# shivangchopra11/MedMoE

Hardware: AMD Instinct MI355X
Metric: image-text pairs/sec at global batch 1024 (higher is better)
Workload: dtype bf16; 1 GPU; cfg2: ViT-B/16 + 12-layer text tower (frozen), 8 experts top-2, 224x224x3 + 77 tokens, fwd+bwd+clip+Adam; global_batch=1024, per_gpu_batch=1024, parallelism=dp1

## Files before the change

### medmoe_amd/csrc/gemm.hip

```cpp
#include "common.h"
#include "det_plan.h"
#include <utility>

#define BM 128
#define BN 128
#define BK 64

__device__ __attribute__((aligned(256))) bf16_t g_zero_page[2048];

struct GemmNTArgs {
  const bf16_t* A; const bf16_t* B; void* C;
  const float* bias; const bf16_t* residual; bf16_t* aux;
  const int* a_rowmap; const int* c_rowmap; const int4* tiles; const int* tile_count;
  long long strideB; long long strideBias;
  int M, N, K, lda, ldb, ldc, ldr, ldaux;
  int n_tiles_n, max_tiles_m;
  float alpha; int epi; int out_f32; int col_perm;
  const int* m_dev;
};

static int g_use_nt256 = 1, g_use_nt512 = 1, g_use_tn512 = 1, g_tn_rows = 1024, g_nt_max_grid = 256, g_use_scores512 = 1, g_use_nt4w = 1, g_use_tn4w = 1, g_tn_min_rows = 2048, g_tn_rows4w = 0, g_scores_skip_epi = 0;
#ifdef NT_EXPERIMENT
__device__ int g_nt_dbg_skip = 0;
#define NT_X(...) __VA_ARGS__
#else
#define NT_X(...)
#endif
#ifdef NT_TIMING
__device__ unsigned long long g_nt_timing[8 * 8];
#define NT_T(...) __VA_ARGS__
__device__ __forceinline__ long long nt_clk() {
  __builtin_amdgcn_sched_barrier(0); const long long c = clock64(); __builtin_amdgcn_sched_barrier(0); return c;
}
#else
#define NT_T(...)
#endif
extern int g_attn_resident;
extern int g_sa_rows;
extern int g_attn_rt13;
static int g_last_nt_kernel = -1;
extern "C" int medmoe_last_gemm_nt_kernel() { return g_last_nt_kernel; }
extern int g_ln_one_row;
int g_use_nt_direct = 1;
extern "C" int medmoe_set_option(int key, int value) {
  if (key == 16) { g_ln_one_row = value; return MM_OK; }
  if (key == 17) { g_use_nt_direct = value; return MM_OK; }
  if (key == 1) { g_use_nt256 = value; return MM_OK; }
  if (key == 2) { g_use_nt512 = value; return MM_OK; }
  if (key == 3) { g_use_tn512 = value; return MM_OK; }
  if (key == 4 && value >= 256) { g_tn_rows = value; return MM_OK; }
  if (key == 5 && value >= 1 && value <= 256) { g_nt_max_grid = value; return MM_OK; }
  if (key == 6) { g_use_scores512 = value; return MM_OK; }
  if (key == 7) { g_use_nt4w = value; return MM_OK; }
  if (key == 8) { g_use_tn4w = value; return MM_OK; }
  if (key == 9 && value >= 64) { g_tn_min_rows = value; return MM_OK; }
  if (key == 12) { g_scores_skip_epi = value; return MM_OK; }
  if (key == 15 && (value == 0 || value == 448 || value == 512)) { g_attn_rt13 = value; return MM_OK; }
  if (key == 13 && value >= 0) { g_sa_rows = value; return MM_OK; }
  if (key == 11) { g_attn_resident = value; return MM_OK; }
  if (key == 10 && value >= 0) { g_tn_rows4w = value; return MM_OK; }
  return MM_ERR_ARG;
}

enum { EPI_NONE = 0, EPI_GELU = 1, EPI_RELU = 2, EPI_MUL_DGELU = 3, EPI_MUL_DRELU = 4, EPI_GELU_DAUX = 5, EPI_MUL_AUX = 6 };

struct ParkedTile {
  uint4 c[8];
  int m_base, n_base, n_items, next;
};

typedef unsigned u32x4e_t __attribute__((ext_vector_type(4)));
template <bool PARK, int TM0 = 0, int TMS = 4, int TN0 = 0, int TNS = 4, bool LDSX = false>
__device__ __forceinline__ int nt_epilogue(const GemmNTArgs& p, f32x4_t (&acc)[TMS][TNS], int m_base, int m_end,
                                           int n_base, int group, int frag_row, int frag_q, ParkedTile* park, unsigned lds_x = 0u) {
  int n_stores = 0;
  const int pg = ((frag_q & 1) << 1) | (frag_q >> 1);
  long long mc[4];
  bool mok[4];
#pragma unroll
  for (int tm = 0; tm < 4; ++tm) {
    const int m = m_base + tm * 16 + frag_row;
    mok[tm] = m < m_end;
    const int mr = min(m, m_end - 1);
    mc[tm] = p.c_rowmap ? (long long)p.c_rowmap[mr] : (long long)mr;
  }
  int nn[4];
  bool nok[4];
#pragma unroll
  for (int tn = 0; tn < 4; ++tn) {
    const int n = n_base + tn * 16 + pg * 4;
    nok[tn] = n < p.N;
    nn[tn] = min(n, p.N - 4);
// ... 1985 lines not shown
  for (int u = 0; u < U; ++u) {
    compute();
    if (grp == 0) { wait_third_newest(); seg_barrier(); }
    if (grp == 1) seg_barrier();
    load_seg();
  }
  if (grp == 0) seg_barrier();

  float* dW = p.dW + (MAPPED ? (long long)group * p.strideW : 0ll);
  const int kcol = lane & 31;
#pragma unroll
  for (int tn = 0; tn < 4; ++tn)
#pragma unroll
    for (int tk = 0; tk < 2; ++tk) {
      const int k = k0 + wn * 64 + tk * 32 + kcol;
#pragma unroll
      for (int r = 0; r < 16; ++r) {
        const int n = n0 + wm * 128 + tn * 32 + (r & 3) + 8 * (r >> 2) + 4 * h;
        if (!MAPPED || n < p.Nn) atomicAdd(dW + (long long)n * p.ldw + k, acc[tn][tk][r]);
      }
    }
  if (do_db) {
#pragma unroll
    for (int tn = 0; tn < 4; ++tn) {
      const float v = colsum[tn] + __shfl_xor(colsum[tn], 32, 64);
      const int n = n0 + wm * 128 + tn * 32 + kcol;
      if (h == 0 && (!MAPPED || n < p.Nn)) atomicAdd(p.db + (MAPPED ? (long long)group * p.strideDb : 0ll) + n, v);
    }
  }
}

typedef unsigned u32x4_t __attribute__((ext_vector_type(4)));
#define W_READ(dst, addr, imm) asm volatile("ds_read_b128 %0, %1 offset:%2" : "=v"(dst) : "v"(addr), "n"(imm))
template <bool MAPPED, bool COLG = false, bool SCALE = false>
__global__ __launch_bounds__(256) void gemm_tn4w_kernel(GemmTNArgs p) {
  static_assert(!(MAPPED && COLG), "column groups only in the plain build");
  static_assert(!SCALE || COLG, "row weights only in the column-group build");
  __shared__ __attribute__((aligned(128))) char smem[4 * SUB3 + (MAPPED ? 32768 : 0) + (SCALE ? 4096 : 0)];
  const int tid = threadIdx.x, lane = tid & 63, wid = __builtin_amdgcn_readfirstlane(tid >> 6);
  const int wm = wid & 1, wn = wid >> 1;
  int id = xcd_remap(blockIdx.x, gridDim.x);
  const int ntile = p.tiles_n * p.tiles_k;
  int group = 0, ms, me;
  if (MAPPED && p.row_off) {
    const int tile = id % ntile;
    if (!det_plan::tn_group_range(p.row_off, p.n_groups, p.nsplit, id / ntile, group, ms, me)) return;
    id = tile;
  } else {
    if (COLG) { group = id / (ntile * p.nsplit); id -= group * ntile * p.nsplit; }
    const int split = id / ntile; id -= split * ntile;
    det_plan::tn_split_range(p.M, p.nsplit, split, ms, me);
  }
  const int tile_n = id / p.tiles_k, tile_k = id - tile_n * p.tiles_k;
  if (ms >= me) return;
  const int U = (me - ms + 31) / 32;
  const int tail = (me - ms) - (U - 1) * 32;
  const int n0 = tile_n * 256, k0 = tile_k * 256;

  const int prow = (wid << 1) + (lane >> 5);
  const unsigned lds0 = (unsigned)(size_t)smem;
  unsigned col_g, col_x;
  {
    const int lc0 = (lane & 31) ^ ((prow & 3) << 2);
    const int gcol = n0 + lc0 * 8;
    col_g = (unsigned)(((MAPPED || COLG) && gcol >= p.Nn) ? n0 : gcol) * 2u;
    if (COLG && p.g_chunk_w > 0) {
      const int gc = (gcol >= p.Nn) ? n0 : gcol;
      const int c0 = n0 / p.g_chunk_w, cc = gc / p.g_chunk_w;
      col_g = (unsigned)((long long)(cc - c0) * p.g_chunk_stride + (gc - cc * p.g_chunk_w)) * 2u;
    }
    const int xcol = k0 + lc0 * 8;
    col_x = (unsigned)((COLG && xcol >= p.Kk) ? k0 : xcol) * 2u;
  }
  const int* rmap = MAPPED ? (p.g_rowmap ? p.g_rowmap : p.x_rowmap) : nullptr;
  int* lmap = (int*)(smem + 4 * SUB3);
  if (MAPPED && rmap) {
    for (int i = tid; i < min(me - ms, 8192); i += 256) lmap[i] = rmap[ms + i];
    __syncthreads();
  }
  const unsigned ldg2 = (unsigned)p.ldg * 2u, ldx2 = (unsigned)p.ldx * 2u;
  int lk = 0, wb = 0, rb = 0;
  unsigned sg[4], sx[4];
  const char* gbase = (const char*)p.G + (COLG ? (long long)group * p.gcol_stride * 2 : 0ll)
                      + ((COLG && p.g_chunk_w > 0) ? (long long)(n0 / p.g_chunk_w) * p.g_chunk_stride * 2 : 0ll);
  const char* xbase = (const char*)p.X + (COLG ? (long long)group * p.xcol_stride * 2 : 0ll);
  const char* gsub = gbase;
  const char* xsub = xbase;
  const char* wbase = SCALE ? (const char*)(p.gscale + (long long)group * p.gscale_gstride) : nullptr;
  const char* wsub = wbase;
  int wr0 = 0;
  const unsigned wl0 = lds0 + 4 * SUB3 + wid * 1024;
  auto setup_rows = [&]() __attribute__((always_inline)) {
    if constexpr (!MAPPED) {
      const long long r0 = ms + min(lk, (me - ms) / 32 - 1) * 32;
      auto uni = [](const char* q) -> const char* {
        const unsigned long long v = (unsigned long long)q;
// ... 75 lines not shown
  };
  auto read_one = [&](Frags& f, unsigned bo, auto gc) __attribute__((always_inline)) {
    constexpr int g = decltype(gc)::value, t = (g >> 2) & 3, ks = (g >> 1) & 1, hi = g & 1;
    constexpr int off = ks * 8192 + hi * 2048;
    const unsigned a = aa[(g < 16 ? 0 : 4) + t] + bo;
    if constexpr (g < 16) { if constexpr (hi) TR_READ(f.gh[ks][t], a, off); else TR_READ(f.gl[ks][t], a, off); }
    else { if constexpr (hi) TR_READ(f.xh[ks][t], a, off); else TR_READ(f.xl[ks][t], a, off); }
  };
  auto frag = [&](u32x2_t lo, u32x2_t hi) -> bf16x8_t {
    const uint4 v = make_uint4(lo[0], lo[1], hi[0], hi[1]);
    return __builtin_bit_cast(bf16x8_t, v);
  };
  auto add_colsum = [&](Frags& f) __attribute__((always_inline)) {
    const s16x2_t ones = {(short)0x3F80, (short)0x3F80};
#pragma unroll
    for (int ks = 0; ks < 2; ++ks)
#pragma unroll
      for (int tn = 0; tn < 4; ++tn) {
        const uint4 v = __builtin_bit_cast(uint4, frag(f.gl[ks][tn], f.gh[ks][tn]));
        float c = colsum[tn];
        c = __builtin_amdgcn_fdot2_f32_bf16(__builtin_bit_cast(s16x2_t, v.x), ones, c, false);
        c = __builtin_amdgcn_fdot2_f32_bf16(__builtin_bit_cast(s16x2_t, v.y), ones, c, false);
        c = __builtin_amdgcn_fdot2_f32_bf16(__builtin_bit_cast(s16x2_t, v.z), ones, c, false);
        c = __builtin_amdgcn_fdot2_f32_bf16(__builtin_bit_cast(s16x2_t, v.w), ones, c, false);
        colsum[tn] = c;
      }
  };
  int u_now = 0;
  auto zero_tail = [&](int buf) __attribute__((always_inline)) {
    char* zb = smem + buf * SUB3;
    for (int z = tail * 32 + lane; z < 32 * 32; z += 64) *(uint4*)(zb + z * 16) = make_uint4(0, 0, 0, 0);
    asm volatile("s_waitcnt lgkmcnt(0)" ::: "memory");
  };
  auto substep = [&](Frags& c, Frags& n) __attribute__((always_inline)) {
    const unsigned bo = rb * SUB3;
    if (MAPPED && rmap && u_now >= 128 && (u_now & 127) == 0) {
      for (int i = tid; i < 4096; i += 256) {
        const int r = (u_now + 128) * 32 + i;
        if (r < me - ms) lmap[r & 8191] = rmap[ms + r];
      }
    }
    if (MAPPED && u_now + 1 == U - 1 && tail < 32) zero_tail(rb);
    if (do_db && (u_now & 1) == wn) add_colsum(c);
    auto one = [&](auto qc) __attribute__((always_inline)) {
      constexpr int qq = decltype(qc)::value, ks = qq >> 4, tn = (qq >> 2) & 3, tk = qq & 3;
      acc[tn][tk] = __builtin_amdgcn_mfma_f32_32x32x16_bf16(frag(c.gl[ks][tn], c.gh[ks][tn]), frag(c.xl[ks][tk], c.xh[ks][tk]), acc[tn][tk], 0, 0, 0);
      if constexpr (qq < 24) {
        __builtin_amdgcn_sched_barrier(0);
        if constexpr (qq < 8) { read_one(n, bo, std::integral_constant<int, 2 * qq>{}); read_one(n, bo, std::integral_constant<int, 2 * qq + 1>{}); }
        else read_one(n, bo, std::integral_constant<int, qq + 8>{});
        if constexpr (qq % 3 == 2) piece(qq / 3);
        if constexpr (SCALE && qq == 0) wpiece();
        if constexpr (SCALE && qq % 4 == 0) scale_frag(c, std::integral_constant<int, qq / 4 + 1>{});
        __builtin_amdgcn_sched_barrier(0);
      }
      if constexpr (SCALE && qq == 24) {
        __builtin_amdgcn_sched_barrier(0);
        scale_frag(c, std::integral_constant<int, 7>{});
        read_w(rb);
        __builtin_amdgcn_sched_barrier(0);
      }
      if constexpr (SCALE && qq == 28) {
        __builtin_amdgcn_sched_barrier(0);
        scale_frag(n, std::integral_constant<int, 0>{});
        __builtin_amdgcn_sched_barrier(0);
      }
// ... 58 lines not shown
      for (int tk = 0; tk < 4; ++tk)
#pragma unroll
        for (int r = 0; r < 16; ++r) part[((tn * 4 + tk) * 16 + r) * 64] = acc[tn][tk][r];
  } else {
#pragma unroll
  for (int tn = 0; tn < 4; ++tn)
#pragma unroll
    for (int tk = 0; tk < 4; ++tk) {
      const int k = k0 + wn * 128 + tk * 32 + kcol;
#pragma unroll
      for (int r = 0; r < 16; ++r) {
        const int n = n0 + wm * 128 + tn * 32 + (r & 3) + 8 * (r >> 2) + 4 * h;
        if ((!(MAPPED || COLG) || n < p.Nn) && (!COLG || k < p.Kk)) atomicAdd(dW + (long long)n * p.ldw + k, acc[tn][tk][r]);
      }
    }
  }
  if (do_db) {
    const bool db_staged = staged && p.db_partial != nullptr;
#pragma unroll
    for (int tn = 0; tn < 4; ++tn) {
      const float v = colsum[tn] + __shfl_xor(colsum[tn], 32, 64);
      const int n = n0 + wm * 128 + tn * 32 + kcol;
      if (db_staged) {
        if (h == 0) p.db_partial[((long long)pid << 9) + (wid << 7) + tn * 32 + kcol] = v;
      } else if (h == 0 && (!(MAPPED || COLG) || n < p.Nn)) atomicAdd(p.db + ((MAPPED || COLG) ? (long long)group * p.strideDb : 0ll) + n, v);
    }
  }
}

extern "C" int medmoe_gemm_tn(const void* G, int ldg, const void* X, int ldx, float* dW, int ldw, float* db, int M, int Nn, int Kk,
                              const int* x_rowmap, const int* g_rowmap, const int* row_off, int n_groups, long long strideW,
                              long long strideDb, int nsplit, hipStream_t stream);

__global__ __launch_bounds__(256) void tn_reduce_kernel(const float* __restrict__ partial, float* __restrict__ dW, int ldw, int ntile,
                                                        int tiles_k, int nvalid) {
  const int tile = blockIdx.x >> 6;
  const int e4 = (((blockIdx.x & 63) << 8) + threadIdx.x) << 2;
  float4 s = {0.f, 0.f, 0.f, 0.f};
  for (int sp = 0; sp < nvalid; ++sp) {
    const float4 v = *(const float4*)(partial + ((long long)(sp * ntile + tile) << 16) + e4);
    s.x += v.x; s.y += v.y; s.z += v.z; s.w += v.w;
  }
  const int lane = e4 & 63, r = (e4 >> 6) & 15, tk = (e4 >> 10) & 3, tn = (e4 >> 12) & 3, wid = e4 >> 14;
  const int wm = wid & 1, wn = wid >> 1, h = lane >> 5, kcol = lane & 31;
  const int tile_n = tile / tiles_k, tile_k = tile - tile_n * tiles_k;
  const int n = tile_n * 256 + wm * 128 + tn * 32 + (r & 3) + 8 * (r >> 2) + 4 * h;
  const int k = tile_k * 256 + wn * 128 + tk * 32 + kcol;
  float4* d = (float4*)(dW + (long long)n * ldw + k);
  float4 o = *d;
  o.x += s.x; o.y += s.y; o.z += s.z; o.w += s.w;
  *d = o;
}

struct TnReduceArgs {
  const float* partial; const float* db_partial; float* dW; float* db; const int* row_off;
  long long strideW, strideDb;
  int ldw, Nn, Kk, tiles_n, tiles_k, mode, nsplit, nvalid, n_groups, R, vec;
};
__global__ __launch_bounds__(256) void tn_reduce_det_kernel(TnReduceArgs p) {
  const int ntile = p.tiles_n * p.tiles_k;
  const int gt = blockIdx.x >> 6;
  const int group = gt / ntile, tile = gt - group * ntile;
  int first, count;
  if (p.mode == 0) { first = group * p.nsplit; count = p.nvalid; }
  else det_plan::tn_group_ranges(p.row_off, group, p.R, first, count);
  const int e4 = (((blockIdx.x & 63) << 8) + threadIdx.x) << 2;
  float4 s = {0.f, 0.f, 0.f, 0.f};
  for (int sp = 0; sp < count; ++sp) {
    const float4 v = *(const float4*)(p.partial + ((long long)((first + sp) * ntile + tile) << 16) + e4);
    s.x += v.x; s.y += v.y; s.z += v.z; s.w += v.w;
  }
  const int lane = e4 & 63, r = (e4 >> 6) & 15, tk = (e4 >> 10) & 3, tn = (e4 >> 12) & 3, wid = e4 >> 14;
  const int wm = wid & 1, wn = wid >> 1, h = lane >> 5, kcol = lane & 31;
  const int tile_n = tile / p.tiles_k, tile_k = tile - tile_n * p.tiles_k;
  const int n = tile_n * 256 + wm * 128 + tn * 32 + (r & 3) + 8 * (r >> 2) + 4 * h;
  const int k = tile_k * 256 + wn * 128 + tk * 32 + kcol;
  if (count > 0 && n < p.Nn && k < p.Kk) {
    float* d = p.dW + (long long)group * p.strideW + (long long)n * p.ldw + k;
    if (p.vec) {
      float4 o = *(float4*)d;
      o.x += s.x; o.y += s.y; o.z += s.z; o.w += s.w;
      *(float4*)d = o;
    } else { d[0] += s.x; d[1] += s.y; d[2] += s.z; d[3] += s.w; }
  }
  if (p.db && tile_k == 0 && (blockIdx.x & 63) == 0 && count > 0) {
    const int c = threadIdx.x;
    const int nn = tile_n * 256 + c;
    float a = 0.f;
    for (int sp = 0; sp < count; ++sp) {
      const float* q = p.db_partial + ((long long)((first + sp) * ntile + tile) << 9) + ((c >> 7) << 7) + (c & 127);
      a += q[0];
      a += q[256];
    }
    if (nn < p.Nn) p.db[(long long)group * p.strideDb + nn] += a;
  }
}

static inline bool tn_vec_ok(const float* dW, int ldw, long long strideW) {
  return ((unsigned long long)dW & 15) == 0 && (ldw % 4) == 0 && (strideW % 4) == 0;
}

extern "C" int medmoe_gemm_tn_staged(const void* G, int ldg, const void* X, int ldx, float* dW, int ldw, float* db, int M, int Nn, int Kk,
                                     float* scratch, long long scratch_floats, hipStream_t stream) {
  if (!G || !X || !dW) return MM_ERR_ARG;
  if (M <= 0 || Nn <= 0 || Kk <= 0 || (Nn % 8) || (Kk % 8) || (ldg % 8) || (ldx % 8)) return MM_ERR_SHAPE;
  const bool fit32 = (long long)M * ldg * 2 < (1ll << 32) && (long long)M * ldx * 2 < (1ll << 32);
  if (scratch && g_use_tn512 && g_use_tn4w && (M % 32) == 0 && (Nn % 256) == 0 && (Kk % 256) == 0 && M >= 4096 && fit32 && (ldw % 4) == 0) {
    GemmTNArgs p;
    p.partial = nullptr;
    p.G = (const bf16_t*)G; p.X = (const bf16_t*)X; p.dW = dW; p.db = db;
    p.x_rowmap = nullptr; p.g_rowmap = nullptr; p.row_off = nullptr; p.strideW = 0; p.strideDb = 0;
    p.M = M; p.Nn = Nn; p.Kk = Kk; p.ldg = ldg; p.ldx = ldx; p.ldw = ldw; p.gcol_stride = 0; p.xcol_stride = 0; p.g_chunk_w = 0; p.g_chunk_stride = 0;
    p.gscale = nullptr; p.gscale_gstride = 0; p.gscale_ld = 0;
    p.tiles_n = Nn / 256; p.tiles_k = Kk / 256;
    const int ntile = p.tiles_n * p.tiles_k;
    p.nsplit = max(1, min(256 / ntile, M / g_tn_min_rows));
    p.n_groups = 1;
    if (p.nsplit >= 2 && (long long)ntile * p.nsplit * 65536 <= scratch_floats) {
      p.partial = scratch;
      const int chunk = det_plan::tn_chunk(M, p.nsplit);
      const int nvalid = (M + chunk - 1) / chunk;
      const long long slots = (long long)ntile * p.nsplit;
      if (db && slots * (65536 + 512) <= scratch_floats) p.db_partial = scratch + slots * 65536;
      if (db && !p.db_partial) ++g_mm_nondet;
      hipLaunchKernelGGL(gemm_tn4w_kernel<false>, dim3(ntile * p.nsplit), dim3(256), 0, stream, p);
      if (p.db_partial) {
        TnReduceArgs q{scratch, p.db_partial, dW, db, nullptr, 0, 0, ldw, Nn, Kk, p.tiles_n, p.tiles_k, 0, p.nsplit, nvalid, 1, 0, 1};
        q.vec = tn_vec_ok(dW, ldw, 0);
        hipLaunchKernelGGL(tn_reduce_det_kernel, dim3(ntile * 64), dim3(256), 0, stream, q);
      } else {
        hipLaunchKernelGGL(tn_reduce_kernel, dim3(ntile * 64), dim3(256), 0, stream, scratch, dW, ldw, ntile, p.tiles_k, nvalid);
      }
      return mm_check_launch();
    }
  }
  return medmoe_gemm_tn(G, ldg, X, ldx, dW, ldw, db, M, Nn, Kk, nullptr, nullptr, nullptr, 1, 0, 0, 16, stream);
}

static int tn_cols_impl(const void* G, int ldg, const void* X, int ldx, float* dW, int ldw, int M, int Nn, int Kk,
                        int n_groups, long long gcol_stride, long long xcol_stride, long long strideW, int g_chunk_w,
                        long long g_chunk_stride, bool det, float* scratch, long long scratch_floats, hipStream_t stream) {
  if (!G || !X || !dW) return MM_ERR_ARG;
  if (M < 32 || (M % 32) || Nn <= 0 || Kk <= 0 || (Nn % 8) || (Kk % 8) || (ldg % 8) || (ldx % 8) || n_groups < 1) return MM_ERR_SHAPE;
  if ((gcol_stride % 8) || (xcol_stride % 8) || gcol_stride < 0 || xcol_stride < 0) return MM_ERR_SHAPE;
  if (32ll * ldg * 2 + 1024 >= (1ll << 32) || 32ll * ldx * 2 + 1024 >= (1ll << 32)) return MM_ERR_SHAPE;
  if ((g_chunk_w <= 0 && Nn > ldg) || Kk > ldx) return MM_ERR_SHAPE;
  if (g_chunk_w > 0 && ((g_chunk_w % 8) || g_chunk_w > ldg || (g_chunk_stride % 8) || g_chunk_stride < 0 ||
                        (256 / g_chunk_w + 2) * g_chunk_stride * 2 + 32ll * ldg * 2 >= (1ll << 32))) return MM_ERR_SHAPE;
  GemmTNArgs p;
  p.partial = nullptr;
  p.G = (const bf16_t*)G; p.X = (const bf16_t*)X; p.dW = dW; p.db = nullptr;
  p.x_rowmap = nullptr; p.g_rowmap = nullptr; p.row_off = nullptr; p.strideW = strideW; p.strideDb = 0;
  p.M = M; p.Nn = Nn; p.Kk = Kk; p.ldg = ldg; p.ldx = ldx; p.ldw = ldw;
  p.tiles_n = (Nn + 255) / 256; p.tiles_k = (Kk + 255) / 256;
  p.n_groups = n_groups; p.gcol_stride = gcol_stride; p.xcol_stride = xcol_stride;
  p.g_chunk_w = g_chunk_w; p.g_chunk_stride = g_chunk_stride;
  p.gscale = nullptr; p.partial = nullptr; p.gscale_gstride = 0; p.gscale_ld = 0;
  const long long ntile = (long long)p.tiles_n * p.tiles_k * n_groups;
  p.nsplit = (int)max(1ll, min(256ll / ntile, (long long)M / g_tn_min_rows));
  if (det && p.nsplit > 1) {
    if (!scratch || ntile * p.nsplit * 65536 > scratch_floats) return MM_ERR_ARG;
    p.partial = scratch;
    const int chunk = det_plan::tn_chunk(M, p.nsplit);
    hipLaunchKernelGGL((gemm_tn4w_kernel<false, true>), dim3((unsigned)(ntile * p.nsplit)), dim3(256), 0, stream, p);
    TnReduceArgs q{scratch, nullptr, dW, nullptr, nullptr, strideW, 0, ldw, Nn, Kk, p.tiles_n, p.tiles_k, 0, p.nsplit, (M + chunk - 1) / chunk,
                   n_groups, 0, tn_vec_ok(dW, ldw, strideW) ? 1 : 0};
    hipLaunchKernelGGL(tn_reduce_det_kernel, dim3((unsigned)(ntile * 64)), dim3(256), 0, stream, q);
    return mm_check_launch();
  }
  if (p.nsplit > 1) ++g_mm_nondet;
  hipLaunchKernelGGL((gemm_tn4w_kernel<false, true>), dim3((unsigned)(ntile * p.nsplit)), dim3(256), 0, stream, p);
  return mm_check_launch();
}

extern "C" int medmoe_gemm_tn_cols(const void* G, int ldg, const void* X, int ldx, float* dW, int ldw, int M, int Nn, int Kk,
                                   int n_groups, long long gcol_stride, long long xcol_stride, long long strideW, int g_chunk_w,
                                   long long g_chunk_stride, hipStream_t stream) {
  return tn_cols_impl(G, ldg, X, ldx, dW, ldw, M, Nn, Kk, n_groups, gcol_stride, xcol_stride, strideW, g_chunk_w, g_chunk_stride, false,
                      nullptr, 0, stream);
}

extern "C" int medmoe_gemm_tn_cols_det(const void* G, int ldg, const void* X, int ldx, float* dW, int ldw, int M, int Nn, int Kk,
                                       int n_groups, long long gcol_stride, long long xcol_stride, long long strideW, int g_chunk_w,
                                       long long g_chunk_stride, float* scratch, long long scratch_floats, hipStream_t stream) {
  return tn_cols_impl(G, ldg, X, ldx, dW, ldw, M, Nn, Kk, n_groups, gcol_stride, xcol_stride, strideW, g_chunk_w, g_chunk_stride, true,
                      scratch, scratch_floats, stream);
}

extern "C" long long medmoe_gemm_tn_cols_det_scratch(int M, int Nn, int Kk, int n_groups) {
  return det_plan::cols_scratch_floats(M, Nn, Kk, n_groups, g_tn_min_rows);
}

static int tn_gram_impl(const void* A, int lda, const float* w, long long w_gstride, int w_ld, float* dW, int ldw, int M,
                        int Nn, int n_groups, long long col_stride, long long strideW, bool det, hipStream_t stream) {
  if (!A || !w || !dW) return MM_ERR_ARG;
  if (M < 32 || (M % 32) || Nn <= 0 || (Nn % 8) || (lda % 8) || n_groups < 1 || Nn > lda || w_ld < 1 || w_gstride < 0) return MM_ERR_SHAPE;
  if ((col_stride % 8) || col_stride < 0 || 32ll * lda * 2 + 1024 >= (1ll << 32) || 64ll * w_ld * 4 >= (1ll << 32)) return MM_ERR_SHAPE;
  GemmTNArgs p;
  p.partial = nullptr;
  p.G = (const bf16_t*)A; p.X = (const bf16_t*)A; p.dW = dW; p.db = nullptr;
  p.x_rowmap = nullptr; p.g_rowmap = nullptr; p.row_off = nullptr; p.strideW = strideW; p.strideDb = 0;
  p.M = M; p.Nn = Nn; p.Kk = Nn; p.ldg = lda; p.ldx = lda; p.ldw = ldw;
  p.tiles_n = (Nn + 255) / 256; p.tiles_k = p.tiles_n;
  p.n_groups = n_groups; p.gcol_stride = col_stride; p.xcol_stride = col_stride;
  p.g_chunk_w = 0; p.g_chunk_stride = 0;
  p.gscale = w; p.gscale_gstride = w_gstride; p.gscale_ld = w_ld;
  const long long ntile = (long long)p.tiles_n * p.tiles_k * n_groups;
  p.nsplit = det ? 1 : (int)max(1ll, min(256ll / ntile, (long long)M / g_tn_min_rows));
  if (p.nsplit > 1) ++g_mm_nondet;
  hipLaunchKernelGGL((gemm_tn4w_kernel<false, true, true>), dim3((unsigned)(ntile * p.nsplit)), dim3(256), 0, stream, p);
  return mm_check_launch();
}

extern "C" int medmoe_gemm_tn_gram(const void* A, int lda, const float* w, long long w_gstride, int w_ld, float* dW, int ldw, int M,
                                   int Nn, int n_groups, long long col_stride, long long strideW, hipStream_t stream) {
  return tn_gram_impl(A, lda, w, w_gstride, w_ld, dW, ldw, M, Nn, n_groups, col_stride, strideW, false, stream);
}

extern "C" int medmoe_gemm_tn_gram_det(const void* A, int lda, const float* w, long long w_gstride, int w_ld, float* dW, int ldw, int M,
                                       int Nn, int n_groups, long long col_stride, long long strideW, hipStream_t stream) {
  return tn_gram_impl(A, lda, w, w_gstride, w_ld, dW, ldw, M, Nn, n_groups, col_stride, strideW, true, stream);
}

extern "C" int medmoe_gemm_tn(const void* G, int ldg, const void* X, int ldx, float* dW, int ldw,
                              float* db, int M, int Nn, int Kk, const int* x_rowmap,
                              const int* g_rowmap, const int* row_off, int n_groups, long long strideW,
                              long long strideDb, int nsplit, hipStream_t stream) {
  if (!G || !X || !dW) return MM_ERR_ARG;
  if (M <= 0 || Nn <= 0 || Kk <= 0 || (Nn % 8) || (Kk % 8) || (ldg % 8) || (ldx % 8)) return MM_ERR_SHAPE;
  if (n_groups < 1 || nsplit < 1) return MM_ERR_ARG;
  GemmTNArgs p;
  p.partial = nullptr;
  p.G = (const bf16_t*)G; p.X = (const bf16_t*)X; p.dW = dW; p.db = db;
  p.x_rowmap = x_rowmap; p.g_rowmap = g_rowmap; p.row_off = row_off; p.strideW = strideW; p.strideDb = strideDb;
  p.M = M; p.Nn = Nn; p.Kk = Kk; p.ldg = ldg; p.ldx = ldx; p.ldw = ldw; p.gcol_stride = 0; p.xcol_stride = 0; p.g_chunk_w = 0; p.g_chunk_stride = 0; p.gscale = nullptr; p.partial = nullptr; p.gscale_gstride = 0; p.gscale_ld = 0;
  const bool fit32 = (long long)M * ldg * 2 < (1ll << 32) && (long long)M * ldx * 2 < (1ll << 32);
  if (g_use_tn512 && !x_rowmap && !g_rowmap && !row_off && n_groups == 1 && (M % 32) == 0 && (Nn % 256) == 0 && (Kk % 256) == 0 &&
      M >= 4096 && fit32) {
    p.tiles_n = Nn / 256; p.tiles_k = Kk / 256;
    const int ntile = p.tiles_n * p.tiles_k;
    p.nsplit = max(1, min(256 / ntile, M / g_tn_min_rows));
    p.n_groups = 1;
    if (p.nsplit > 1) ++g_mm_nondet;
    if (g_use_tn4w) hipLaunchKernelGGL(gemm_tn4w_kernel<false>, dim3(ntile * p.nsplit), dim3(256), 0, stream, p);
    else hipLaunchKernelGGL(gemm_tn512_kernel<false>, dim3(ntile * p.nsplit), dim3(512), 0, stream, p);
    return mm_check_launch();
  }
  if (g_use_tn512 && !(x_rowmap && g_rowmap) && (Nn % 128) == 0 && (Kk % 256) == 0 && M / n_groups >= 4096 && fit32) {
    p.tiles_n = (Nn + 255) / 256; p.tiles_k = Kk / 256;
    const int ntile = p.tiles_n * p.tiles_k;
    p.n_groups = n_groups;
    ++g_mm_nondet;
    if (g_use_tn4w && row_off) {
      long long R = g_tn_rows4w > 0 ? (g_tn_rows4w + 31) / 32 * 32 : 4096;
      p.nsplit = (int)R;
      const int max_ranges = (int)(M / R) + n_groups;
      hipLaunchKernelGGL(gemm_tn4w_kernel<true>, dim3(ntile * max_ranges), dim3(256), 0, stream, p);
      return mm_check_launch();
    }
    p.nsplit = max(1, M / n_groups / g_tn_rows);
    if (g_use_tn4w) hipLaunchKernelGGL(gemm_tn4w_kernel<true>, dim3(ntile * p.nsplit * n_groups), dim3(256), 0, stream, p);
    else hipLaunchKernelGGL(gemm_tn512_kernel<true>, dim3(ntile * p.nsplit * n_groups), dim3(512), 0, stream, p);
    return mm_check_launch();
  }
  p.tiles_n = (Nn + 127) / 128; p.tiles_k = (Kk + 127) / 128; p.nsplit = nsplit; p.n_groups = n_groups;
  if (nsplit > 1) ++g_mm_nondet;
  const int grid = p.tiles_n * p.tiles_k * nsplit * n_groups;
  if (x_rowmap || g_rowmap) hipLaunchKernelGGL(gemm_tn_kernel<true>, dim3(grid), dim3(256), 0, stream, p);
  else hipLaunchKernelGGL(gemm_tn_kernel<false>, dim3(grid), dim3(256), 0, stream, p);
  return mm_check_launch();
}

extern "C" int medmoe_gemm_tn_det(const void* G, int ldg, const void* X, int ldx, float* dW, int ldw, float* db, int M, int Nn, int Kk,
                                  const int* x_rowmap, const int* g_rowmap, const int* row_off, int n_groups, long long strideW,
                                  long long strideDb, float* scratch, long long scratch_floats, hipStream_t stream) {
  if (!G || !X || !dW) return MM_ERR_ARG;
  if (M <= 0 || Nn <= 0 || Kk <= 0 || (Nn % 8) || (Kk % 8) || (ldg % 8) || (ldx % 8)) return MM_ERR_SHAPE;
  if (n_groups < 1 || (n_groups > 1 && !row_off)) return MM_ERR_ARG;
  GemmTNArgs p;
  p.G = (const bf16_t*)G; p.X = (const bf16_t*)X; p.dW = dW; p.db = db;
  p.x_rowmap = x_rowmap; p.g_rowmap = g_rowmap; p.row_off = row_off; p.strideW = strideW; p.strideDb = strideDb;
  p.M = M; p.Nn = Nn; p.Kk = Kk; p.ldg = ldg; p.ldx = ldx; p.ldw = ldw; p.gcol_stride = 0; p.xcol_stride = 0; p.g_chunk_w = 0; p.g_chunk_stride = 0;
  p.gscale = nullptr; p.partial = nullptr; p.gscale_gstride = 0; p.gscale_ld = 0; p.n_groups = n_groups;
  const bool fit32 = (long long)M * ldg * 2 < (1ll << 32) && (long long)M * ldx * 2 < (1ll << 32);
  const det_plan::TnPlan pl = det_plan::tn_plan(M, Nn, Kk, x_rowmap != nullptr, g_rowmap != nullptr, row_off != nullptr, n_groups, fit32,
                                               g_tn_min_rows, g_tn_rows4w);
  if (pl.kind == det_plan::TN_SMALL) {
    p.tiles_n = (Nn + 127) / 128; p.tiles_k = (Kk + 127) / 128; p.nsplit = 1;
    const int grid = p.tiles_n * p.tiles_k * n_groups;
    if (x_rowmap || g_rowmap) hipLaunchKernelGGL(gemm_tn_kernel<true>, dim3(grid), dim3(256), 0, stream, p);
    else hipLaunchKernelGGL(gemm_tn_kernel<false>, dim3(grid), dim3(256), 0, stream, p);
    return mm_check_launch();
  }
  if (!scratch || pl.scratch_floats > scratch_floats) return MM_ERR_ARG;
  p.tiles_n = pl.tiles_n; p.tiles_k = pl.tiles_k; p.nsplit = pl.nsplit;
  const int ntile = pl.tiles_n * pl.tiles_k;
  p.partial = scratch;
  if (db) p.db_partial = scratch + (long long)pl.slots * 65536;
  TnReduceArgs q{scratch, p.db_partial, dW, db, row_off, strideW, strideDb, ldw, Nn, Kk, pl.tiles_n, pl.tiles_k, 0, pl.nsplit, pl.nvalid,
                 n_groups, 0, tn_vec_ok(dW, ldw, strideW) ? 1 : 0};
  if (pl.kind == det_plan::TN_PLAIN) hipLaunchKernelGGL(gemm_tn4w_kernel<false>, dim3(pl.slots), dim3(256), 0, stream, p);
  else {
    if (pl.kind == det_plan::TN_GROUPS) { q.mode = 1; q.R = pl.nsplit; }
    hipLaunchKernelGGL(gemm_tn4w_kernel<true>, dim3(pl.slots), dim3(256), 0, stream, p);
  }
  hipLaunchKernelGGL(tn_reduce_det_kernel, dim3((unsigned)(n_groups * ntile * 64)), dim3(256), 0, stream, q);
  return mm_check_launch();
}

extern "C" long long medmoe_gemm_tn_det_scratch(int M, int Nn, int Kk, int x_mapped, int g_mapped, int grouped, int n_groups) {
  return det_plan::tn_plan(M, Nn, Kk, x_mapped != 0, g_mapped != 0, grouped != 0, n_groups, true, g_tn_min_rows, g_tn_rows4w).scratch_floats;
}

__attribute__((visibility("hidden"))) long long g_mm_nondet = 0;
extern "C" long long medmoe_nondet_launches() { return g_mm_nondet; }
```

Before: 4800 pairs/s.

## Add 16x16x32 MFMA k-loop variant for TN weight-gradient GEMM scaled build

Adds an alternate inner loop to the TN (weight-gradient) GEMM kernel that uses v_mfma_f32_16x16x32_bf16 with 8x8 (or 7x7 for small scaled shapes) tiles of 16 per wave instead of 32x32x16. It comes with a new LDS swizzle, an interleaved read and prefetch schedule, and a matching partial-sum layout in the reduce kernels. By default only the scaled column-group build uses the new path, with a 7x7 specialisation for tiles up to 224 wide. The goal is better MFMA throughput and less waste on the router/gating weight-gradient shapes. The cost is higher register pressure and a hand-tuned schedule that could stall.

```diff
diff --git a/medmoe_amd/csrc/gemm.hip b/medmoe_amd/csrc/gemm.hip
--- a/medmoe_amd/csrc/gemm.hip
+++ b/medmoe_amd/csrc/gemm.hip
@@ -35,6 +35,7 @@
 #else
 #define NT_T(...)
 #endif
+static void tn_shape_set(int build, int s16);
 extern int g_attn_resident;
 extern int g_sa_rows;
 extern int g_attn_rt13;
@@ -58,6 +59,10 @@
   if (key == 15 && (value == 0 || value == 448 || value == 512)) { g_attn_rt13 = value; return MM_OK; }
   if (key == 13 && value >= 0) { g_sa_rows = value; return MM_OK; }
   if (key == 11) { g_attn_resident = value; return MM_OK; }
+  if (key == 18 && ((value >= 0 && value <= 2) || (value >= 16 && value < 32))) {
+    for (int i = 0; i < 4; ++i) tn_shape_set(i, value >= 16 ? (value >> i) & 1 : value == 2 ? -1 : value);
+    return MM_OK;
+  }
   if (key == 10 && value >= 0) { g_tn_rows4w = value; return MM_OK; }
   return MM_ERR_ARG;
 }
@@ -2109,10 +2114,11 @@
 
 typedef unsigned u32x4_t __attribute__((ext_vector_type(4)));
 #define W_READ(dst, addr, imm) asm volatile("ds_read_b128 %0, %1 offset:%2" : "=v"(dst) : "v"(addr), "n"(imm))
-template <bool MAPPED, bool COLG = false, bool SCALE = false>
+template <bool MAPPED, bool COLG = false, bool SCALE = false, int S16 = 0>
 __global__ __launch_bounds__(256) void gemm_tn4w_kernel(GemmTNArgs p) {
   static_assert(!(MAPPED && COLG), "column groups only in the plain build");
   static_assert(!SCALE || COLG, "row weights only in the column-group build");
+  static_assert(S16 == 0 || S16 == 8 || (S16 == 7 && SCALE), "k-loop body: 0 = 32x32x16, 8 / 7 = 16x16x32 with 8 x 8 / 7 x 7 tiles of 16 per wave");
   __shared__ __attribute__((aligned(128))) char smem[4 * SUB3 + (MAPPED ? 32768 : 0) + (SCALE ? 4096 : 0)];
   const int tid = threadIdx.x, lane = tid & 63, wid = __builtin_amdgcn_readfirstlane(tid >> 6);
   const int wm = wid & 1, wn = wid >> 1;
@@ -2138,7 +2144,7 @@
   const unsigned lds0 = (unsigned)(size_t)smem;
   unsigned col_g, col_x;
   {
-    const int lc0 = (lane & 31) ^ ((prow & 3) << 2);
+    const int lc0 = (lane & 31) ^ ((prow & 3) << 2) ^ (S16 ? ((prow >> 2) & 1) << 1 : 0);
     const int gcol = n0 + lc0 * 8;
     col_g = (unsigned)(((MAPPED || COLG) && gcol >= p.Nn) ? n0 : gcol) * 2u;
     if (COLG && p.g_chunk_w > 0) {
@@ -2280,6 +2286,224 @@
     for (int z = tail * 32 + lane; z < 32 * 32; z += 64) *(uint4*)(zb + z * 16) = make_uint4(0, 0, 0, 0);
     asm volatile("s_waitcnt lgkmcnt(0)" ::: "memory");
   };
+  if constexpr (S16 != 0) {
+    constexpr int NT = S16, NE = 2 * NT + 4;
+    constexpr int PG = NT == 8 ? 6 : 4;
+    constexpr int QA = NT * (NT - 2) + 3, QW = QA + 5;
+    static_assert(NE <= QA && 8 * PG - 1 < QA && QW + 2 < NT * NT, "every read and piece before the wait");
+    f32x4_t ac[NT][NT];
+#pragma unroll
+    for (int i = 0; i < NT; ++i)
+#pragma unroll
+      for (int j = 0; j < NT; ++j) ac[i][j] = (f32x4_t){0.f, 0.f, 0.f, 0.f};
+    float cs[NT];
+#pragma unroll
+    for (int i = 0; i < NT; ++i) cs[i] = 0.f;
+    const int g4 = lane >> 4;
+    unsigned ag[NT], ax[NT == 8 ? 1 : NT];
+#pragma unroll
+    for (int t = 0; t < NT; ++t) {
+      const int sw = (q << 2) ^ ((g4 & 1) << 1);
+      const int cg = (NT == 8 ? 0 : wm * 2 * NT) + t * 2 + (pp >> 1), cx = wn * 2 * NT + t * 2 + (pp >> 1);
+      const unsigned ro = (unsigned)(4 * g4 + q) * 512u + ((pp & 1) << 3);
+      ag[t] = lds0 + ro + ((cg ^ sw) << 4);
+      if constexpr (NT != 8) ax[t] = lds0 + ro + ((cx ^ sw) << 4);
+    }
+    const unsigned sg16 = NT == 8 ? wm * 256 : 0, sx16 = 16384 + (NT == 8 ? wn * 256 : 0);
+    struct GS16 { u32x2_t gb[2][NT], ge[2][2]; };
+    GS16 gs;
+    u32x2_t xa[2][NT], xb[2][NT];
+#define G16_CUR(f, P, hf, t) (((P) == 1 && (t) >= NT - 2) ? f.ge[hf][(t) - (NT - 2)] : f.gb[hf][(t)])
+#define G16_NXT(f, P, hf, t) (((P) == 0 && (t) >= NT - 2) ? f.ge[hf][(t) - (NT - 2)] : f.gb[hf][(t)])
+    u32x4_t w16[2];
+    const unsigned wa16 = wl0 + 16 * g4;
+    auto read_w16 = [&](int buf) __attribute__((always_inline)) {
+      if constexpr (SCALE) { const unsigned a = wa16 + buf * 256; W_READ(w16[0], a, 0); W_READ(w16[1], a, 64); }
+    };
+    auto scale16 = [&](GS16& f, auto pc, auto nc, auto ic) __attribute__((always_inline)) {
+      if constexpr (SCALE) {
+        constexpr int P = decltype(pc)::value ^ decltype(nc)::value, tn = decltype(ic)::value;
+        auto sc = [](unsigned v, unsigned w0, unsigned w1) -> unsigned {
+          return pack2bf(__uint_as_float(v << 16) * __uint_as_float(w0), __uint_as_float(v & 0xffff0000u) * __uint_as_float(w1));
+        };
+#pragma unroll
+        for (int hf = 0; hf < 2; ++hf) {
+          u32x2_t& v = G16_CUR(f, P, hf, tn);
+          v[0] = sc(v[0], w16[hf][0], w16[hf][1]);
+          v[1] = sc(v[1], w16[hf][2], w16[hf][3]);
+        }
+      }
+    };
+    auto read_g16 = [&](GS16& f, auto pc, unsigned bo, auto tc, auto hc) __attribute__((always_inline)) {
+      constexpr int P = decltype(pc)::value, t = decltype(tc)::value, hf = decltype(hc)::value;
+      const unsigned a = ag[t] + (bo + sg16);
+      TR_READ(G16_NXT(f, P, hf, t), a, hf * 8192);
+    };
+    auto read_x16 = [&](u32x2_t (&xn)[2][NT], unsigned bo, auto tc, auto hc) __attribute__((always_inline)) {
+      constexpr int t = decltype(tc)::value, hf = decltype(hc)::value;
+      const unsigned a = (NT == 8 ? ag[t] : ax[t]) + (bo + sx16);
+      TR_READ(xn[hf][t], a, hf * 8192);
+    };
+    auto read_early = [&](GS16& f, auto pc, u32x2_t (&xn)[2][NT], unsigned bo, auto ec) __attribute__((always_inline)) {
+      constexpr int e = decltype(ec)::value;
+      if constexpr (e < 2 * NT) read_x16(xn, bo, std::integral_constant<int, (e >> 1)>{}, std::integral_constant<int, (e & 1)>{});
+      else read_g16(f, pc, bo, std::integral_constant<int, NT - 2 + ((e - 2 * NT) >> 1)>{}, std::integral_constant<int, (e & 1)>{});
+    };
+    auto colsum16 = [&](GS16& f, auto pc) __attribute__((always_inline)) {
+      constexpr int P = decltype(pc)::value;
+      const s16x2_t ones = {(short)0x3F80, (short)0x3F80};
+#pragma unroll
+      for (int tn = 0; tn < NT; ++tn) {
+        const uint4 v = __builtin_bit_cast(uint4, frag(G16_CUR(f, P, 0, tn), G16_CUR(f, P, 1, tn)));
+        float c = cs[tn];
+        c = __builtin_amdgcn_fdot2_f32_bf16(__builtin_bit_cast(s16x2_t, v.x), ones, c, false);
+        c = __builtin_amdgcn_fdot2_f32_bf16(__builtin_bit_cast(s16x2_t, v.y), ones, c, false);
+        c = __builtin_amdgcn_fdot2_f32_bf16(__builtin_bit_cast(s16x2_t, v.z), ones, c, false);
+        c = __builtin_amdgcn_fdot2_f32_bf16(__builtin_bit_cast(s16x2_t, v.w), ones, c, false);
+        cs[tn] = c;
+      }
+    };
+    auto piece16 = [&](int i) __attribute__((always_inline)) {
+      if constexpr (MAPPED) piece(i);
+      else {
+        const char* b = (i < 4 ? gsub : xsub) + (unsigned long long)(8 * (i & 3)) * (i < 4 ? ldg2 : ldx2);
+        __builtin_amdgcn_global_load_lds(GLB_PTR(b + (i < 4 ? sg[0] : sx[0])),
+                                         (__attribute__((address_space(3))) void*)(size_t)(ldsW + i * 4096), 16, 0, 0);
+      }
+    };
+    const bool do_db16 = !COLG && do_db;
+    auto substep16 = [&](GS16& f, auto pc, u32x2_t (&xc)[2][NT], u32x2_t (&xn)[2][NT]) __attribute__((always_inline)) {
+      constexpr int P = decltype(pc)::value;
+      const unsigned bo = rb * SUB3;
+      if (MAPPED && rmap && u_now >= 128 && (u_now & 127) == 0) {
+        for (int i = tid; i < 4096; i += 256) {
+          const int r = (u_now + 128) * 32 + i;
+          if (r < me - ms) lmap[r & 8191] = rmap[ms + r];
+        }
+      }
+      if (MAPPED && u_now + 1 == U - 1 && tail < 32) zero_tail(rb);
+      if (do_db16 && (u_now & 1) == wn) colsum16(f, pc);
+      auto one = [&](auto qc) __attribute__((always_inline)) {
+        constexpr int qq = decltype(qc)::value, tn = qq / NT, tk = qq % NT;
+        {
+          const bf16x8_t fa = frag(G16_CUR(f, P, 0, tn), G16_CUR(f, P, 1, tn)), fb = frag(xc[0][tk], xc[1][tk]);
+          asm volatile("v_mfma_f32_16x16x32_bf16 %0, %1, %2, %0" : "+a"(ac[tn][tk]) : "v"(fa), "v"(fb));
+        }
+        constexpr bool re = qq < NE;
+        constexpr bool rl = tk == 0 && tn >= 1 && tn - 1 < NT - 2;
+        constexpr bool dp = qq % PG == PG - 1 && qq / PG < 8;
+        constexpr bool sc = SCALE && tk == 0 && tn + 1 < NT;
+        if constexpr (re || rl || dp || sc) {
+          __builtin_amdgcn_sched_barrier(0);
+          if constexpr (re) read_early(f, pc, xn, bo, std::integral_constant<int, (re ? qq : 0)>{});
+          if constexpr (rl) {
+            read_g16(f, pc, bo, std::integral_constant<int, (rl ? tn - 1 : 0)>{}, std::integral_constant<int, 0>{});
+            read_g16(f, pc, bo, std::integral_constant<int, (rl ? tn - 1 : 0)>{}, std::integral_constant<int, 1>{});
+          }
+          if constexpr (dp) piece16(qq / PG);
+          if constexpr (SCALE && qq == 0) wpiece();
+          if constexpr (sc) scale16(f, pc, std::integral_constant<int, 0>{}, std::integral_constant<int, (tn + 1) % NT>{});
+          if constexpr (sc && tn + 2 == NT) read_w16(rb);
+          __builtin_amdgcn_sched_barrier(0);
+        }
+        if constexpr (SCALE && qq == QW + 1) {
+          __builtin_amdgcn_sched_barrier(0);
+          scale16(f, pc, std::integral_constant<int, 1>{}, std::integral_constant<int, 0>{});
+          __builtin_amdgcn_sched_barrier(0);
+        }
+        if constexpr (qq == QA) { advance(); rb = (rb + 1) & 3; ++u_now; }
+        if constexpr (qq == QW) {
+          __builtin_amdgcn_sched_barrier(0);
+          asm volatile("s_waitcnt lgkmcnt(0)\n\ts_waitcnt vmcnt(16)" ::: "memory");
+          __builtin_amdgcn_s_barrier();
+          __builtin_amdgcn_sched_barrier(0);
+          asm volatile("" ::: "memory");
+        }
+      };
+      static_for<NT * NT>(one);
+    };
+
+    setup_rows();
+    for (int v = 0; v < 4; ++v) {
+      wpiece();
+#pragma unroll
+      for (int i = 0; i < 8; ++i) piece16(i);
+      advance();
+    }
+    asm volatile("s_waitcnt vmcnt(24)" ::: "memory");
+    __builtin_amdgcn_s_barrier();
+    asm volatile("" ::: "memory");
+    if (MAPPED && U == 1 && tail < 32) zero_tail(0);
+    {
+      auto rd = [&](auto tc) __attribute__((always_inline)) {
+        read_g16(gs, std::integral_constant<int, 1>{}, 0u, tc, std::integral_constant<int, 0>{});
+        read_g16(gs, std::integral_constant<int, 1>{}, 0u, tc, std::integral_constant<int, 1>{});
+        read_x16(xa, 0u, tc, std::integral_constant<int, 0>{});
+        read_x16(xa, 0u, tc, std::integral_constant<int, 1>{});
+      };
+      static_for<NT>(rd);
+      read_w16(0);
+    }
+    rb = 1;
+    asm volatile("s_waitcnt lgkmcnt(0)\n\ts_waitcnt vmcnt(16)" ::: "memory");
+    __builtin_amdgcn_s_barrier();
+    __builtin_amdgcn_sched_barrier(0);
+    asm volatile("" ::: "memory");
+    scale16(gs, std::integral_constant<int, 0>{}, std::integral_constant<int, 0>{}, std::integral_constant<int, 0>{});
+    int u = 0;
+    for (; u + 1 < U; u += 2) { substep16(gs, std::integral_constant<int, 0>{}, xa, xb); substep16(gs, std::integral_constant<int, 1>{}, xb, xa); }
+    if (u < U) substep16(gs, std::integral_constant<int, 0>{}, xa, xb);
+    asm volatile("s_waitcnt vmcnt(0)\n\ts_nop 15\n\ts_nop 15" ::: "memory");
+    if constexpr (SCALE) asm volatile("" :: "v"(w16[0]), "v"(w16[1]));
+    asm volatile("s_waitcnt lgkmcnt(0)" ::: "memory");
+#pragma unroll
+    for (int hf = 0; hf < 2; ++hf) {
+#pragma unroll
+      for (int t = 0; t < NT; ++t) asm volatile("" :: "v"(gs.gb[hf][t]), "v"(xa[hf][t]), "v"(xb[hf][t]));
+      asm volatile("" :: "v"(gs.ge[hf][0]), "v"(gs.ge[hf][1]));
+    }
+#undef G16_CUR
+#undef G16_NXT
+
+    float* dW = p.dW + ((MAPPED || COLG) ? (long long)group * p.strideW : 0ll);
+    const int kc = lane & 15;
+    const bool staged = p.partial != nullptr;
+    const int pid = staged ? xcd_remap(blockIdx.x, gridDim.x) : 0;
+    if (staged) {
+      float* part = p.partial + ((long long)pid << 16) + (wid << 14) + lane;
+#pragma unroll
+      for (int tn = 0; tn < NT; ++tn)
+#pragma unroll
+        for (int tk = 0; tk < NT; ++tk)
+#pragma unroll
+          for (int r = 0; r < 4; ++r) part[((tn * 8 + tk) * 4 + r) * 64] = ac[tn][tk][r];
+    } else {
+#pragma unroll
+      for (int tn = 0; tn < NT; ++tn)
+#pragma unroll
+        for (int tk = 0; tk < NT; ++tk) {
+          const int k = k0 + wn * 16 * NT + tk * 16 + kc;
+#pragma unroll
+          for (int r = 0; r < 4; ++r) {
+            const int n = n0 + wm * 16 * NT + tn * 16 + 4 * g4 + r;
+            if ((!(MAPPED || COLG) || n < p.Nn) && (!COLG || k < p.Kk)) atomicAdd(dW + (long long)n * p.ldw + k, ac[tn][tk][r]);
+          }
+        }
+    }
+    if (do_db16) {
+      const bool db_staged = staged && p.db_partial != nullptr;
+#pragma unroll
+      for (int tn = 0; tn < NT; ++tn) {
+        float v = cs[tn] + __shfl_xor(cs[tn], 16, 64);
+        v += __shfl_xor(v, 32, 64);
+        const int n = n0 + wm * 16 * NT + tn * 16 + kc;
+        if (db_staged) {
+          if (g4 == 0) p.db_partial[((long long)pid << 9) + (wid << 7) + tn * 16 + kc] = v;
+        } else if (g4 == 0 && (!(MAPPED || COLG) || n < p.Nn)) atomicAdd(p.db + ((MAPPED || COLG) ? (long long)group * p.strideDb : 0ll) + n, v);
+      }
+    }
+    return;
+  }
   auto substep = [&](Frags& c, Frags& n) __attribute__((always_inline)) {
     const unsigned bo = rb * SUB3;
     if (MAPPED && rmap && u_now >= 128 && (u_now & 127) == 0) {
@@ -2404,8 +2628,20 @@
                               const int* x_rowmap, const int* g_rowmap, const int* row_off, int n_groups, long long strideW,
                               long long strideDb, int nsplit, hipStream_t stream);
 
+__device__ __forceinline__ void tn_partial_rc(int e4, int s16, int& n, int& k) {
+  const int lane = e4 & 63, wid = e4 >> 14, wm = wid & 1, wn = wid >> 1;
+  if (s16) {
+    const int r = (e4 >> 6) & 3, tk = (e4 >> 8) & 7, tn = (e4 >> 11) & 7;
+    n = wm * 128 + tn * 16 + 4 * (lane >> 4) + r;
+    k = wn * 128 + tk * 16 + (lane & 15);
+  } else {
+    const int r = (e4 >> 6) & 15, tk = (e4 >> 10) & 3, tn = (e4 >> 12) & 3, h = lane >> 5, kcol = lane & 31;
+    n = wm * 128 + tn * 32 + (r & 3) + 8 * (r >> 2) + 4 * h;
+    k = wn * 128 + tk * 32 + kcol;
+  }
+}
 __global__ __launch_bounds__(256) void tn_reduce_kernel(const float* __restrict__ partial, float* __restrict__ dW, int ldw, int ntile,
-                                                        int tiles_k, int nvalid) {
+                                                        int tiles_k, int nvalid, int s16) {
   const int tile = blockIdx.x >> 6;
   const int e4 = (((blockIdx.x & 63) << 8) + threadIdx.x) << 2;
   float4 s = {0.f, 0.f, 0.f, 0.f};
@@ -2413,11 +2649,10 @@
     const float4 v = *(const float4*)(partial + ((long long)(sp * ntile + tile) << 16) + e4);
     s.x += v.x; s.y += v.y; s.z += v.z; s.w += v.w;
   }
-  const int lane = e4 & 63, r = (e4 >> 6) & 15, tk = (e4 >> 10) & 3, tn = (e4 >> 12) & 3, wid = e4 >> 14;
-  const int wm = wid & 1, wn = wid >> 1, h = lane >> 5, kcol = lane & 31;
   const int tile_n = tile / tiles_k, tile_k = tile - tile_n * tiles_k;
-  const int n = tile_n * 256 + wm * 128 + tn * 32 + (r & 3) + 8 * (r >> 2) + 4 * h;
-  const int k = tile_k * 256 + wn * 128 + tk * 32 + kcol;
+  int n, k;
+  tn_partial_rc(e4, s16, n, k);
+  n += tile_n * 256; k += tile_k * 256;
   float4* d = (float4*)(dW + (long long)n * ldw + k);
   float4 o = *d;
   o.x += s.x; o.y += s.y; o.z += s.z; o.w += s.w;
@@ -2428,7 +2663,25 @@
   const float* partial; const float* db_partial; float* dW; float* db; const int* row_off;
   long long strideW, strideDb;
   int ldw, Nn, Kk, tiles_n, tiles_k, mode, nsplit, nvalid, n_groups, R, vec;
+  int s16;
 };
+
+static const int g_tn_shape_default[4] = {0, 0, 0, 1};
+static int g_tn_shape[4] = {g_tn_shape_default[0], g_tn_shape_default[1], g_tn_shape_default[2], g_tn_shape_default[3]};
+static void tn_shape_set(int build, int s16) { g_tn_shape[build] = s16 < 0 ? g_tn_shape_default[build] : s16; }
+template <bool MAPPED, bool COLG, bool SCALE>
+static int launch_tn4w(unsigned grid, hipStream_t stream, const GemmTNArgs& p) {
+  const int s = g_tn_shape[SCALE ? 3 : COLG ? 2 : MAPPED ? 1 : 0];
+  if constexpr (SCALE) {
+    if (s && p.tiles_n == 1 && p.tiles_k == 1 && p.Nn <= 224 && p.Kk <= 224) {
+      hipLaunchKernelGGL((gemm_tn4w_kernel<MAPPED, COLG, SCALE, 7>), dim3(grid), dim3(256), 0, stream, p);
+      return 1;
+    }
+  }
+  if (s) hipLaunchKernelGGL((gemm_tn4w_kernel<MAPPED, COLG, SCALE, 8>), dim3(grid), dim3(256), 0, stream, p);
+  else hipLaunchKernelGGL((gemm_tn4w_kernel<MAPPED, COLG, SCALE, 0>), dim3(grid), dim3(256), 0, stream, p);
+  return s ? 1 : 0;
+}
 __global__ __launch_bounds__(256) void tn_reduce_det_kernel(TnReduceArgs p) {
   const int ntile = p.tiles_n * p.tiles_k;
   const int gt = blockIdx.x >> 6;
@@ -2442,11 +2695,10 @@
     const float4 v = *(const float4*)(p.partial + ((long long)((first + sp) * ntile + tile) << 16) + e4);
     s.x += v.x; s.y += v.y; s.z += v.z; s.w += v.w;
   }
-  const int lane = e4 & 63, r = (e4 >> 6) & 15, tk = (e4 >> 10) & 3, tn = (e4 >> 12) & 3, wid = e4 >> 14;
-  const int wm = wid & 1, wn = wid >> 1, h = lane >> 5, kcol = lane & 31;
   const int tile_n = tile / p.tiles_k, tile_k = tile - tile_n * p.tiles_k;
-  const int n = tile_n * 256 + wm * 128 + tn * 32 + (r & 3) + 8 * (r >> 2) + 4 * h;
-  const int k = tile_k * 256 + wn * 128 + tk * 32 + kcol;
+  int n, k;
+  tn_partial_rc(e4, p.s16, n, k);
+  n += tile_n * 256; k += tile_k * 256;
   if (count > 0 && n < p.Nn && k < p.Kk) {
     float* d = p.dW + (long long)group * p.strideW + (long long)n * p.ldw + k;
     if (p.vec) {
@@ -2495,13 +2747,13 @@
       const long long slots = (long long)ntile * p.nsplit;
       if (db && slots * (65536 + 512) <= scratch_floats) p.db_partial = scratch + slots * 65536;
       if (db && !p.db_partial) ++g_mm_nondet;
-      hipLaunchKernelGGL(gemm_tn4w_kernel<false>, dim3(ntile * p.nsplit), dim3(256), 0, stream, p);
+      const int s16 = launch_tn4w<false, false, false>(ntile * p.nsplit, stream, p);
       if (p.db_partial) {
         TnReduceArgs q{scratch, p.db_partial, dW, db, nullptr, 0, 0, ldw, Nn, Kk, p.tiles_n, p.tiles_k, 0, p.nsplit, nvalid, 1, 0, 1};
-        q.vec = tn_vec_ok(dW, ldw, 0);
+        q.vec = tn_vec_ok(dW, ldw, 0); q.s16 = s16;
         hipLaunchKernelGGL(tn_reduce_det_kernel, dim3(ntile * 64), dim3(256), 0, stream, q);
       } else {
-        hipLaunchKernelGGL(tn_reduce_kernel, dim3(ntile * 64), dim3(256), 0, stream, scratch, dW, ldw, ntile, p.tiles_k, nvalid);
+        hipLaunchKernelGGL(tn_reduce_kernel, dim3(ntile * 64), dim3(256), 0, stream, scratch, dW, ldw, ntile, p.tiles_k, nvalid, s16);
       }
       return mm_check_launch();
     }
@@ -2534,14 +2786,15 @@
     if (!scratch || ntile * p.nsplit * 65536 > scratch_floats) return MM_ERR_ARG;
     p.partial = scratch;
     const int chunk = det_plan::tn_chunk(M, p.nsplit);
-    hipLaunchKernelGGL((gemm_tn4w_kernel<false, true>), dim3((unsigned)(ntile * p.nsplit)), dim3(256), 0, stream, p);
+    const int s16 = launch_tn4w<false, true, false>((unsigned)(ntile * p.nsplit), stream, p);
     TnReduceArgs q{scratch, nullptr, dW, nullptr, nullptr, strideW, 0, ldw, Nn, Kk, p.tiles_n, p.tiles_k, 0, p.nsplit, (M + chunk - 1) / chunk,
                    n_groups, 0, tn_vec_ok(dW, ldw, strideW) ? 1 : 0};
+    q.s16 = s16;
     hipLaunchKernelGGL(tn_reduce_det_kernel, dim3((unsigned)(ntile * 64)), dim3(256), 0, stream, q);
     return mm_check_launch();
   }
   if (p.nsplit > 1) ++g_mm_nondet;
-  hipLaunchKernelGGL((gemm_tn4w_kernel<false, true>), dim3((unsigned)(ntile * p.nsplit)), dim3(256), 0, stream, p);
+  launch_tn4w<false, true, false>((unsigned)(ntile * p.nsplit), stream, p);
   return mm_check_launch();
 }
 
@@ -2580,7 +2833,7 @@
   const long long ntile = (long long)p.tiles_n * p.tiles_k * n_groups;
   p.nsplit = det ? 1 : (int)max(1ll, min(256ll / ntile, (long long)M / g_tn_min_rows));
   if (p.nsplit > 1) ++g_mm_nondet;
-  hipLaunchKernelGGL((gemm_tn4w_kernel<false, true, true>), dim3((unsigned)(ntile * p.nsplit)), dim3(256), 0, stream, p);
+  launch_tn4w<false, true, true>((unsigned)(ntile * p.nsplit), stream, p);
   return mm_check_launch();
 }
 
@@ -2614,7 +2867,7 @@
     p.nsplit = max(1, min(256 / ntile, M / g_tn_min_rows));
     p.n_groups = 1;
     if (p.nsplit > 1) ++g_mm_nondet;
-    if (g_use_tn4w) hipLaunchKernelGGL(gemm_tn4w_kernel<false>, dim3(ntile * p.nsplit), dim3(256), 0, stream, p);
+    if (g_use_tn4w) launch_tn4w<false, false, false>(ntile * p.nsplit, stream, p);
     else hipLaunchKernelGGL(gemm_tn512_kernel<false>, dim3(ntile * p.nsplit), dim3(512), 0, stream, p);
     return mm_check_launch();
   }
@@ -2627,11 +2880,11 @@
       long long R = g_tn_rows4w > 0 ? (g_tn_rows4w + 31) / 32 * 32 : 4096;
       p.nsplit = (int)R;
       const int max_ranges = (int)(M / R) + n_groups;
-      hipLaunchKernelGGL(gemm_tn4w_kernel<true>, dim3(ntile * max_ranges), dim3(256), 0, stream, p);
+      launch_tn4w<true, false, false>(ntile * max_ranges, stream, p);
       return mm_check_launch();
     }
     p.nsplit = max(1, M / n_groups / g_tn_rows);
-    if (g_use_tn4w) hipLaunchKernelGGL(gemm_tn4w_kernel<true>, dim3(ntile * p.nsplit * n_groups), dim3(256), 0, stream, p);
+    if (g_use_tn4w) launch_tn4w<true, false, false>(ntile * p.nsplit * n_groups, stream, p);
     else hipLaunchKernelGGL(gemm_tn512_kernel<true>, dim3(ntile * p.nsplit * n_groups), dim3(512), 0, stream, p);
     return mm_check_launch();
   }
@@ -2671,10 +2924,10 @@
   if (db) p.db_partial = scratch + (long long)pl.slots * 65536;
   TnReduceArgs q{scratch, p.db_partial, dW, db, row_off, strideW, strideDb, ldw, Nn, Kk, pl.tiles_n, pl.tiles_k, 0, pl.nsplit, pl.nvalid,
                  n_groups, 0, tn_vec_ok(dW, ldw, strideW) ? 1 : 0};
-  if (pl.kind == det_plan::TN_PLAIN) hipLaunchKernelGGL(gemm_tn4w_kernel<false>, dim3(pl.slots), dim3(256), 0, stream, p);
+  if (pl.kind == det_plan::TN_PLAIN) q.s16 = launch_tn4w<false, false, false>(pl.slots, stream, p);
   else {
     if (pl.kind == det_plan::TN_GROUPS) { q.mode = 1; q.R = pl.nsplit; }
-    hipLaunchKernelGGL(gemm_tn4w_kernel<true>, dim3(pl.slots), dim3(256), 0, stream, p);
+    q.s16 = launch_tn4w<true, false, false>(pl.slots, stream, p);
   }
   hipLaunchKernelGGL(tn_reduce_det_kernel, dim3((unsigned)(n_groups * ntile * 64)), dim3(256), 0, stream, q);
   return mm_check_launch();
```

Result: no change. 4810 pairs/s, median of 6 (+0.2%).
